# PRBonn/OverlapNet

Measured on AMD Instinct MI355X. Metric: scan-pairs/s (64x900 range images), higher is better.
Workload: dtype f32 (scaled 3-term fp16 split on the fp16 MFMA: 22 significand bits per operand, fp32 accumulate)

## Files before the change

overlapnet_amd/csrc/c3_dense.hip:

```cpp
#include "ovn_internal.h"

typedef _Float16 f16x8 __attribute__((ext_vector_type(8)));
typedef _Float16 f16x4 __attribute__((ext_vector_type(4)));

namespace {

struct ArithF16 {
  typedef _Float16 elem;
  typedef f16x8 v8;
  typedef f16x4 v4;
  static __device__ __forceinline__ f32x4 mfma(v8 a, v8 b, f32x4 c) { return __builtin_amdgcn_mfma_f32_16x16x32_f16(a, b, c, 0, 0, 0); }
};

constexpr int G = OVN_G;
constexpr int OW = OVN_O3_HW;
constexpr int CI = OVN_C2_OUT;
constexpr int CO = OVN_C3_OUT;
constexpr int NBAND = 3;
constexpr int MAX_ROWS = 8;
constexpr int MAX_MT = (MAX_ROWS * OW + 15) / 16;
constexpr int IN_PIX_MAX = (MAX_ROWS + 2) * G;
constexpr int PLANE = IN_PIX_MAX * 8 + 8;
constexpr int NPL = CI / 8;
constexpr size_t LDS_BYTES = 2 * (size_t)NPL * PLANE * sizeof(_Float16) + 64;
constexpr int NW = 8;

__device__ __forceinline__ int band_start(int b) { return b == 0 ? 0 : (b == 1 ? 8 : 15); }
__device__ __forceinline__ int band_rows(int b) { return b == 0 ? 8 : 7; }

constexpr int MT_SPLIT = 6;
template <class A, int NWV, int MSPLIT>
__global__ __launch_bounds__(64 * NWV) void c3_dense_kernel(const float* __restrict__ o2, const typename A::elem* __restrict__ wp,
                                                           const float* __restrict__ b3, const float* __restrict__ wd,
                                                           const unsigned* __restrict__ o2max, float sw3,
                                                           float* __restrict__ partial, float* __restrict__ o3,
                                                           unsigned* __restrict__ arrived, const float* __restrict__ bd,
                                                           float* __restrict__ overlap, float* __restrict__ logit) {
  typedef typename A::elem elem_t;
  typedef typename A::v8 v8_t;
  typedef typename A::v4 v4_t;
  extern __shared__ __attribute__((aligned(16))) unsigned char smem[];
  elem_t* ih = reinterpret_cast<elem_t*>(smem);
  elem_t* il = ih + NPL * PLANE;
  float* red = reinterpret_cast<float*>(il + NPL * PLANE);

  constexpr int HALVES = NW / NWV;
  constexpr int MTW = MSPLIT == 1 ? MAX_MT : MT_SPLIT;
  const int sub = blockIdx.x % (HALVES * MSPLIT);
  const int unit = blockIdx.x / (HALVES * MSPLIT), half = sub % HALVES, mh = sub / HALVES;
  const int mt0 = MT_SPLIT * mh;
  const int pair = unit / NBAND;
  const int band = unit - pair * NBAND;
  const int r0 = band_start(band);
  const int nrows = band_rows(band);
  const int npix = nrows * OW;
  const int nmt = (npix + 15) >> 4;
  const int tid = threadIdx.x;
  const int lane = tid & 63;
  const int wave_l = tid >> 6;
  const int wave = wave_l + NWV * half;
  const int lrow = lane & 15;
  const int g = lane >> 4;

  const elem_t* wsrc = wp + ((size_t)(2 * wave) * 2) * 512 + lane * 8;
  v8_t bq[3][4];
#define C3_LOAD_B(DST, KC)                                                                  \
  {                                                                                         \
    const elem_t* q = wsrc + (size_t)(KC) * (16 * 2 * 512);                                 \
    DST[0] = *reinterpret_cast<const v8_t*>(q);                                           \
    DST[1] = *reinterpret_cast<const v8_t*>(q + 512);                                     \
    DST[2] = *reinterpret_cast<const v8_t*>(q + 1024);                                    \
    DST[3] = *reinterpret_cast<const v8_t*>(q + 1536);                                    \
  }
  C3_LOAD_B(bq[0], 0)
  C3_LOAD_B(bq[1], 1)
  const float s2 = ovn_pow2_scale_for(__uint_as_float(o2max[pair]));
  const float inv = 1.0f / (s2 * sw3);
  {
    const float* src = o2 + ((long long)pair * G + r0) * G * CI;
    const int n4 = (nrows + 2) * G * CI / 4;
    constexpr int PER_THREAD = (MAX_ROWS + 2) * G * CI / 4 / (64 * NWV);
    static_assert(PER_THREAD * 64 * NWV == (MAX_ROWS + 2) * G * CI / 4, "patch does not divide over the threads");
    f32x4 v[PER_THREAD];
#pragma unroll
    for (int k = 0; k < PER_THREAD; ++k) {
      const int i = tid + k * (64 * NWV);
      v[k] = (i < n4) ? *reinterpret_cast<const f32x4*>(src + 4 * i) : (f32x4){0.f, 0.f, 0.f, 0.f};
    }
#pragma unroll
    for (int k = 0; k < PER_THREAD; ++k) {
      const int i = tid + k * (64 * NWV);
      if (i < n4) {
        const int pix = i / (CI / 4);
        const int c = 4 * (i - pix * (CI / 4));
        v4_t h, l;
// ... 58 lines not shown
        C3_READ_A(nb, 1, 2 * q + 3)                                                         \
      } else if (MTW % 2 == 1 && nmt == MAX_MT) {                                                           \
        C3_READ_A(nb, 0, MTW - 1)                                                        \
      }                                                                                     \
      __builtin_amdgcn_sched_barrier(0);   \
      C3_MFMA2(2 * q, 2 * q + 1, fh[cb][0], fl[cb][0], fh[cb][1], fl[cb][1], SRC)           \
      __builtin_amdgcn_sched_barrier(0);                                                    \
    }                                                                                       \
    if (MTW % 2 == 1 && nmt == MAX_MT) {                               \
      const v8_t ah = fh[(MTW / 2) & 1][0], al = fl[(MTW / 2) & 1][0];              \
      acc[MTW - 1][0] = A::mfma(ah, SRC[0], acc[MTW - 1][0]); \
      acc[MTW - 1][1] = A::mfma(ah, SRC[2], acc[MTW - 1][1]); \
      acc[MTW - 1][0] = A::mfma(al, SRC[0], acc[MTW - 1][0]); \
      acc[MTW - 1][1] = A::mfma(al, SRC[2], acc[MTW - 1][1]); \
      acc[MTW - 1][0] = A::mfma(ah, SRC[1], acc[MTW - 1][0]); \
      acc[MTW - 1][1] = A::mfma(ah, SRC[3], acc[MTW - 1][1]); \
    }                                                                                       \
  }
  __syncthreads();
#pragma unroll 1
  for (int kc = 0; kc < 36; kc += 3) {
    C3_LOAD_B(bq[2], kc + 2)
    C3_STEP(bq[0], kc)
    if (kc + 3 < 36) C3_LOAD_B(bq[0], kc + 3)
    C3_STEP(bq[1], kc + 1)
    if (kc + 4 < 36) C3_LOAD_B(bq[1], kc + 4)
    C3_STEP(bq[2], kc + 2)
  }
#undef C3_LOAD_B
#undef C3_STEP
#undef C3_MFMA2
#undef C3_READ_A

  float s[2] = {0.f, 0.f};
#pragma unroll
  for (int nt = 0; nt < 2; ++nt) {
    const int n = 32 * wave + 16 * nt + lrow;
    const float bv = b3[n];
#pragma unroll
    for (int mt = 0; mt < MTW; ++mt) {
#pragma unroll
      for (int r = 0; r < 4; ++r) {
        const int p = 16 * (mt0 + mt) + 4 * g + r;
        if (p < npix) {
          const float v = fmaxf(fmaf(acc[mt][nt][r], inv, bv), 0.0f);
          const long long fi = (long long)(r0 * OW + p) * CO + n;
          s[(MSPLIT == 1 && mt >= MT_SPLIT) ? 1 : 0] += v * wd[fi];
          if (o3) o3[(long long)pair * OVN_DENSE_IN + fi] = v;
        }
      }
    }
  }
#pragma unroll
  for (int off = 32; off > 0; off >>= 1) {
    s[0] += __shfl_down(s[0], off, 64);
    if (MSPLIT == 1) s[1] += __shfl_down(s[1], off, 64);
  }
  if (lane == 0) {
    red[wave_l] = s[0];
    if (MSPLIT == 1) red[NW + wave_l] = s[1];
  }
  __syncthreads();
  if (tid == 0) {
    float* dst = partial + ((size_t)pair * NBAND + band) * 4;
    if (NWV == NW) {
      dst[0] = (red[0] + red[1]) + (red[2] + red[3]);
      dst[1] = (red[NW + 0] + red[NW + 1]) + (red[NW + 2] + red[NW + 3]);
      dst[2] = (red[4] + red[5]) + (red[6] + red[7]);
      dst[3] = (red[NW + 4] + red[NW + 5]) + (red[NW + 6] + red[NW + 7]);
    } else {
      dst[2 * half + mh] = (red[0] + red[1]) + (red[2] + red[3]);
    }
    if (overlap != nullptr) {
      constexpr unsigned PARTS = NBAND * HALVES * MSPLIT;
      __threadfence();
      const unsigned prev = atomicAdd(arrived + pair, 1u);
      if (prev == PARTS - 1) {
        __threadfence();
        const float* q = partial + (size_t)pair * OVN_DENSE_PARTIALS;
        float z = 0.f;
#pragma unroll
        for (int b = 0; b < NBAND; ++b) {
          const float q0 = __hip_atomic_load(q + 4 * b, __ATOMIC_RELAXED, __HIP_MEMORY_SCOPE_AGENT);
          const float q1 = __hip_atomic_load(q + 4 * b + 1, __ATOMIC_RELAXED, __HIP_MEMORY_SCOPE_AGENT);
          const float q2 = __hip_atomic_load(q + 4 * b + 2, __ATOMIC_RELAXED, __HIP_MEMORY_SCOPE_AGENT);
          const float q3 = __hip_atomic_load(q + 4 * b + 3, __ATOMIC_RELAXED, __HIP_MEMORY_SCOPE_AGENT);
          const float zb = (q0 + q1) + (q2 + q3);
          z = b == 0 ? zb : z + zb;
        }
        z += bd[0];
        if (logit) logit[pair] = z;
        overlap[pair] = 1.0f / (1.0f + expf(-z));
        __hip_atomic_store(arrived + pair, 0u, __ATOMIC_RELAXED, __HIP_MEMORY_SCOPE_AGENT);
      }
    }
  }
}

__global__ __launch_bounds__(256) void dense_finish_kernel(const float* __restrict__ partial, const float* __restrict__ bd, int n,
                                                           float* __restrict__ overlap, float* __restrict__ logit) {
  const int p = blockIdx.x * 256 + threadIdx.x;
  if (p >= n) return;
  const float* q = partial + (size_t)p * OVN_DENSE_PARTIALS;
  float z = 0.f;
#pragma unroll
  for (int b = 0; b < NBAND; ++b) {
    const float zb = (q[4 * b] + q[4 * b + 1]) + (q[4 * b + 2] + q[4 * b + 3]);
    z = b == 0 ? zb : z + zb;
  }
  z += bd[0];
  if (logit) logit[p] = z;
  overlap[p] = 1.0f / (1.0f + expf(-z));
}

}

int ovn_c3_dense_forward(const ovn_ctx* ctx, const float* o2, const unsigned* o2max, int n, float* partial, float* o3,
                         unsigned* arrived, float* overlap, float* logit, hipStream_t stream) {
  OVN_REQUIRE(o2max != nullptr, OVN_ERR_ARG, "ovn_c3_dense_forward: the per-pair maxima of o2 are required");
  OVN_REQUIRE(overlap == nullptr || arrived != nullptr, OVN_ERR_ARG, "ovn_c3_dense_forward: arrival counters missing");
  int rc;
  if (n <= 21) {
    rc = ovn_allow_dynamic_lds(reinterpret_cast<const void*>(c3_dense_kernel<ArithF16, 4, 2>), LDS_BYTES);
    if (rc) return rc;
    hipLaunchKernelGGL((c3_dense_kernel<ArithF16, 4, 2>), dim3(4 * NBAND * n), dim3(64 * 4), LDS_BYTES, stream, o2,
                       reinterpret_cast<const _Float16*>(ctx->c3.wp_h), ctx->c3.bias, ctx->wd, o2max, ctx->c3.sw_h, partial, o3, arrived,
                       ctx->bd, overlap, logit);
  } else {
    rc = ovn_allow_dynamic_lds(reinterpret_cast<const void*>(c3_dense_kernel<ArithF16, NW, 1>), LDS_BYTES);
    if (rc) return rc;
    hipLaunchKernelGGL((c3_dense_kernel<ArithF16, NW, 1>), dim3(NBAND * n), dim3(64 * NW), LDS_BYTES, stream, o2,
                       reinterpret_cast<const _Float16*>(ctx->c3.wp_h), ctx->c3.bias, ctx->wd, o2max, ctx->c3.sw_h, partial, o3,
                       (unsigned*)nullptr, ctx->bd, (float*)nullptr, (float*)nullptr);
    if (overlap != nullptr)
      hipLaunchKernelGGL(dense_finish_kernel, dim3((n + 255) / 256), dim3(256), 0, stream, partial, ctx->bd, n, overlap, logit);
  }
  OVN_HIP_CHECK(hipGetLastError());
  return OVN_OK;
}
```

overlapnet_amd/csrc/ovn_api.hip:

```cpp
#include <stdarg.h>
#include <mutex>
#include <set>
#include <utility>
#include <stdio.h>
#include <stdlib.h>
#include <string.h>

#include <algorithm>
#include "ovn_internal.h"

int ovn_allow_dynamic_lds(const void* kernel, size_t bytes) {
  static std::mutex mu;
  static std::set<std::pair<const void*, int>> done;
  int dev = 0;
  OVN_HIP_CHECK(hipGetDevice(&dev));
  std::lock_guard<std::mutex> lock(mu);
  if (done.count({kernel, dev})) return OVN_OK;
  OVN_HIP_CHECK(hipFuncSetAttribute(kernel, hipFuncAttributeMaxDynamicSharedMemorySize, (int)bytes));
  done.insert({kernel, dev});
  return OVN_OK;
}

static thread_local char g_err[1024] = "";

// ... 14 lines not shown
    ctx->dbg_o2 = ctx->dbg_o3 = nullptr;
    ctx->dbg_partial = nullptr;
    ctx->dbg_o2max = nullptr;
    ctx->dbg_n = 0;
    ctx->dbg_live = nullptr;
  }
  const size_t want = bytes + bytes / 8;
  OVN_HIP_CHECK(hipMalloc(&ctx->ws, want));
  ctx->ws_bytes = want;
  return OVN_OK;
}

static int ctx_feat_w(const ovn_ctx* ctx) { return ctx->finalized ? ctx->feat_w : OVN_FEAT_W; }

extern "C" {

int ovn_abi_version(void) { return OVN_ABI_VERSION; }

const char* ovn_last_error(void) { return g_err; }

int ovn_create(int device_id, int in_h, int in_w, int in_c, ovn_ctx** out) {
  OVN_REQUIRE(out != nullptr, OVN_ERR_ARG, "ovn_create: out is NULL");
  OVN_REQUIRE(in_h > 0 && in_w > 0 && in_c > 0, OVN_ERR_ARG, "ovn_create: bad input shape %dx%dx%d", in_h, in_w, in_c);
  int ndev = 0;
  OVN_HIP_CHECK(hipGetDeviceCount(&ndev));
  OVN_REQUIRE(device_id >= 0 && device_id < ndev, OVN_ERR_ARG, "ovn_create: device %d not present (%d devices)", device_id, ndev);
  OVN_ON_DEVICE(device_id);
  hipDeviceProp_t prop;
  OVN_HIP_CHECK(hipGetDeviceProperties(&prop, device_id));
  OVN_REQUIRE(strncmp(prop.gcnArchName, "gfx950", 6) == 0, OVN_ERR_STATE,
              "ovn_create: this library is built for gfx950 only, device %d is %s", device_id, prop.gcnArchName);
  ovn_ctx* c = new ovn_ctx();
  c->device = device_id;
  c->in_h = in_h;
  c->in_w = in_w;
  c->in_c = in_c;
  if (const char* e = getenv("OVN_HEAD_CHUNK")) c->head_chunk = atoll(e) > 0 ? atoll(e) : c->head_chunk;
  if (const char* e = getenv("OVN_HEAD_SUBCHUNK")) c->head_sub = atoll(e) >= 0 ? atoll(e) : c->head_sub;
  if (const char* e = getenv("OVN_HEAD_STREAMS")) c->head_streams = atoi(e) == 2 ? 2 : 1;
  if (const char* e = getenv("OVN_YAW_SIDE")) c->head_yaw_side = atoi(e) ? 1 : 0;
  int rc = ovn_spectral_prepare(c, nullptr);
  if (rc) {
    ovn_conv_release(&c->dft);
    if (c->tw64) (void)hipFree(c->tw64);
    delete c;
    return rc;
  }
  *out = c;
  return OVN_OK;
}

int ovn_destroy(ovn_ctx* ctx) {
  if (!ctx) return OVN_OK;
  if (ctx->comm) (void)ovn_comm_destroy(ctx);
  OVN_ON_DEVICE(ctx->device);
  (void)hipDeviceSynchronize();
  for (auto& l : ctx->leg) ovn_conv_release(&l);
  ovn_conv_release(&ctx->c2);
  ovn_conv_release(&ctx->c3);
  ovn_conv_release(&ctx->dft);
  if (ctx->tw64) (void)hipFree(ctx->tw64);
  if (ctx->w1p) (void)hipFree(ctx->w1p);
  if (ctx->b1) (void)hipFree(ctx->b1);
  if (ctx->wd) (void)hipFree(ctx->wd);
  if (ctx->bd) (void)hipFree(ctx->bd);
  if (ctx->w1p_h) (void)hipFree(ctx->w1p_h);
  if (ctx->w2p_h) (void)hipFree(ctx->w2p_h);
  if (ctx->w1raw) (void)hipFree(ctx->w1raw);
  if (ctx->w1sum) (void)hipFree(ctx->w1sum);
  if (ctx->w1col) (void)hipFree(ctx->w1col);
  if (ctx->wsp_h) (void)hipFree(ctx->wsp_h);
  if (ctx->w2sum) (void)hipFree(ctx->w2sum);
  if (ctx->w1p_b3) (void)hipFree(ctx->w1p_b3);
  if (ctx->w2p_b3) (void)hipFree(ctx->w2p_b3);
  if (ctx->w2raw) (void)hipFree(ctx->w2raw);
  if (ctx->w3raw) (void)hipFree(ctx->w3raw);
  if (ctx->ws) (void)hipFree(ctx->ws);
  if (ctx->norm_buf) (void)hipFree(ctx->norm_buf);
  if (ctx->actmax) (void)hipFree(ctx->actmax);
  if (ctx->c3_arrived) (void)hipFree(ctx->c3_arrived);
  if (ctx->seg_dev) (void)hipFree(ctx->seg_dev);
  if (ctx->seg_host) (void)hipHostFree(ctx->seg_host);
  if (ctx->seg_ev) (void)hipEventDestroy(ctx->seg_ev);
  if (ctx->seg_done) (void)hipEventDestroy(ctx->seg_done);
  if (ctx->aux_ready) {
    for (int i = 0; i < 2; ++i) {
      (void)hipStreamDestroy(ctx->aux[i]);
      (void)hipEventDestroy(ctx->ev_join[i]);
    }
    (void)hipEventDestroy(ctx->ev_fork);
  }
  delete ctx;
  return OVN_OK;
}

static int leg_layer_prepare(OvnConvLayer* L, const float* kernel_dev, const float* bias_dev, hipStream_t stream) {
  int rc = ovn_conv_prepare(L, kernel_dev, bias_dev, stream);
  if (rc == OVN_OK) rc = ovn_conv_prepare_f16x3(L, kernel_dev, stream);
  if (rc == OVN_OK) {
    const size_t bytes = (size_t)L->kh * L->kw * L->cin * L->cout * sizeof(float);
    hipError_t e = hipMalloc((void**)&L->wraw, bytes);
    if (e == hipSuccess) e = hipMemcpyAsync(L->wraw, kernel_dev, bytes, hipMemcpyDeviceToDevice, stream);
    if (e == hipSuccess) e = hipStreamSynchronize(stream);
    if (e != hipSuccess) {
      ovn_set_error("layer %s: keeping the raw kernel failed: %s", L->name.c_str(), hipGetErrorString(e));
      rc = OVN_ERR_HIP;
    }
  }
  if (rc) ovn_conv_release(L);
  return rc;
}

int ovn_add_leg_layer(ovn_ctx* ctx, const char* name, const float* kernel_dev, const float* bias_dev, int kh, int kw,
// ... 17 lines not shown
  int rc = leg_layer_prepare(&L, kernel_dev, bias_dev, (hipStream_t)stream);
  if (rc) return rc;
  ctx->leg.push_back(L);
  return OVN_OK;
}

int ovn_set_leg_layer_weights(ovn_ctx* ctx, int layer, const float* kernel_dev, const float* bias_dev, void* stream) {
  OVN_REQUIRE(ctx && kernel_dev && bias_dev, OVN_ERR_ARG, "ovn_set_leg_layer_weights: NULL argument");
  OVN_REQUIRE(ctx->finalized, OVN_ERR_STATE, "ovn_set_leg_layer_weights: context not finalized");
  OVN_REQUIRE(layer >= 0 && layer < (int)ctx->leg.size(), OVN_ERR_ARG, "ovn_set_leg_layer_weights: no such leg layer %d", layer);
  OVN_ON_DEVICE(ctx->device);
  OvnConvLayer N = ctx->leg[layer];
  N.wp = N.bias = N.wraw = nullptr;
  N.wp_h = N.wp_h16 = nullptr;
  N.sw_h = 1.f;
  int rc = leg_layer_prepare(&N, kernel_dev, bias_dev, (hipStream_t)stream);
  if (rc) return rc;
  ovn_conv_release(&ctx->leg[layer]);
  ctx->leg[layer] = N;
  return OVN_OK;
}

int ovn_set_head_weights(ovn_ctx* ctx, const float* c1k, const float* c1b, const float* c2k, const float* c2b,
                         const float* c3k, const float* c3b, const float* dk, const float* db, void* stream_) {
  OVN_REQUIRE(ctx && c1k && c1b && c2k && c2b && c3k && c3b && dk && db, OVN_ERR_ARG, "ovn_set_head_weights: NULL argument");
  OVN_ON_DEVICE(ctx->device);
  hipStream_t stream = (hipStream_t)stream_;
  {
    ovn_conv_release(&ctx->c2);
    ovn_conv_release(&ctx->c3);
    if (ctx->w1p) (void)hipFree(ctx->w1p);
    if (ctx->b1) (void)hipFree(ctx->b1);
    if (ctx->wd) (void)hipFree(ctx->wd);
    if (ctx->bd) (void)hipFree(ctx->bd);
    if (ctx->w1p_h) (void)hipFree(ctx->w1p_h);
    if (ctx->w2p_h) (void)hipFree(ctx->w2p_h);
    if (ctx->w1raw) (void)hipFree(ctx->w1raw);
    if (ctx->w1sum) (void)hipFree(ctx->w1sum);
    if (ctx->w1col) (void)hipFree(ctx->w1col);
    if (ctx->wsp_h) (void)hipFree(ctx->wsp_h);
      if (ctx->w2sum) (void)hipFree(ctx->w2sum);
    if (ctx->w1p_b3) (void)hipFree(ctx->w1p_b3);
    if (ctx->w2p_b3) (void)hipFree(ctx->w2p_b3);
    if (ctx->w2raw) (void)hipFree(ctx->w2raw);
    if (ctx->w3raw) (void)hipFree(ctx->w3raw);
    ctx->w3raw = nullptr;
    ctx->w1p_h = ctx->w2p_h = ctx->wsp_h = ctx->w1p_b3 = ctx->w2p_b3 = nullptr;
    ctx->w1raw = ctx->w1sum = ctx->w1col = ctx->w2sum = ctx->w2raw = nullptr;
    ctx->w1p = ctx->b1 = ctx->wd = ctx->bd = nullptr;
    ctx->head_set = false;
  }
  ctx->head_g = ctx_feat_w(ctx) / ctx->head_s;
  const int hs = ctx->head_s, hg = ctx->head_g;
  OVN_REQUIRE(hg >= 3, OVN_ERR_ARG, "ovn_set_head_weights: conv1size %d leaves %d column groups, c_conv3 needs 3", hs, hg);
  const bool general = (hs != OVN_S);
  int rc = OVN_OK;
  if (!general) {
    rc = ovn_delta_prepare_w1(c1k, &ctx->w1p, stream);
    if (rc) return rc;
  } else {
    const size_t w1_bytes = (size_t)hs * OVN_FEAT_C * OVN_C1_OUT * sizeof(float);
    OVN_HIP_CHECK(hipMalloc((void**)&ctx->w1raw, w1_bytes));
    OVN_HIP_CHECK(hipMemcpyAsync(ctx->w1raw, c1k, w1_bytes, hipMemcpyDeviceToDevice, stream));
  }
  OVN_HIP_CHECK(hipMalloc((void**)&ctx->b1, OVN_C1_OUT * sizeof(float)));
  OVN_HIP_CHECK(hipMemcpyAsync(ctx->b1, c1b, OVN_C1_OUT * sizeof(float), hipMemcpyDeviceToDevice, stream));
  ctx->c2 = OvnConvLayer();
  ctx->c2.name = "c_conv2";
  ctx->c2.kh = hs;
  ctx->c2.kw = 1;
  ctx->c2.cin = OVN_C1_OUT;
  ctx->c2.cout = OVN_C2_OUT;
  ctx->c2.sh = hs;
  ctx->c2.sw = 1;
  ctx->c2.relu = 1;
  rc = ovn_conv_prepare(&ctx->c2, c2k, c2b, stream);
  if (rc) return rc;
  if (!general) {
    rc = ovn_delta_prepare_f16x3(ctx, c1k, c1b, c2k, stream);
    if (rc) return rc;
  }
  ctx->c3 = OvnConvLayer();
  ctx->c3.name = "c_conv3";
  ctx->c3.kh = 3;
  ctx->c3.kw = 3;
  ctx->c3.cin = OVN_C2_OUT;
  ctx->c3.cout = OVN_C3_OUT;
  ctx->c3.sh = 1;
  ctx->c3.sw = 1;
  ctx->c3.relu = 1;
  rc = ovn_conv_prepare(&ctx->c3, c3k, c3b, stream);
  if (rc) return rc;
  if (!general) {
    rc = ovn_conv_prepare_f16x3(&ctx->c3, c3k, stream);
    if (rc) return rc;
  }
  const size_t w3_bytes = (size_t)9 * OVN_C2_OUT * OVN_C3_OUT * sizeof(float);
  OVN_HIP_CHECK(hipMalloc((void**)&ctx->w3raw, w3_bytes));
  OVN_HIP_CHECK(hipMemcpyAsync(ctx->w3raw, c3k, w3_bytes, hipMemcpyDeviceToDevice, stream));
  if (!ctx->w2raw) {
    const size_t w2_bytes = (size_t)hs * OVN_C1_OUT * OVN_C2_OUT * sizeof(float);
    OVN_HIP_CHECK(hipMalloc((void**)&ctx->w2raw, w2_bytes));
    OVN_HIP_CHECK(hipMemcpyAsync(ctx->w2raw, c2k, w2_bytes, hipMemcpyDeviceToDevice, stream));
  }
  const size_t dense_in = (size_t)(hg - 2) * (hg - 2) * OVN_C3_OUT;
  OVN_HIP_CHECK(hipMalloc((void**)&ctx->wd, dense_in * sizeof(float)));
  OVN_HIP_CHECK(hipMalloc((void**)&ctx->bd, sizeof(float)));
  OVN_HIP_CHECK(hipMemcpyAsync(ctx->wd, dk, dense_in * sizeof(float), hipMemcpyDeviceToDevice, stream));
  OVN_HIP_CHECK(hipMemcpyAsync(ctx->bd, db, sizeof(float), hipMemcpyDeviceToDevice, stream));
  OVN_HIP_CHECK(hipStreamSynchronize(stream));
  ctx->head_set = true;
  return OVN_OK;
}

int ovn_finalize(ovn_ctx* ctx, int* feat_w) {
  OVN_REQUIRE(ctx != nullptr, OVN_ERR_ARG, "ovn_finalize: ctx is NULL");
  OVN_REQUIRE(!ctx->leg.empty(), OVN_ERR_STATE, "ovn_finalize: no leg layers registered");
  int h = ctx->in_h, w = ctx->in_w, c = ctx->in_c;
  for (const auto& l : ctx->leg) {
    OVN_REQUIRE(h >= l.kh && w >= l.kw, OVN_ERR_ARG, "ovn_finalize: layer %s does not fit its %dx%d input", l.name.c_str(), h, w);
    h = (h - l.kh) / l.sh + 1;
    w = (w - l.kw) / l.sw + 1;
    c = l.cout;
  }
  OVN_REQUIRE(h == 1 && w >= OVN_FEAT_W_MIN && w <= OVN_FEAT_W_MAX && c == OVN_FEAT_C, OVN_ERR_ARG,
              "ovn_finalize: leg produces %dx%dx%d, the heads need 1 x W x %d with %d <= W <= %d", h, w, c, OVN_FEAT_C, OVN_FEAT_W_MIN,
              OVN_FEAT_W_MAX);
  OVN_REQUIRE(!ctx->head_set || w / ctx->head_s == ctx->head_g, OVN_ERR_STATE,
              "ovn_finalize: leg width %d gives %d column groups, the head weights were registered for %d", w, w / ctx->head_s,
              ctx->head_g);
  ctx->feat_w = w;
  ctx->finalized = true;
  if (feat_w) *feat_w = w;
  return OVN_OK;
}

int ovn_leg(ovn_ctx* ctx, const float* images_dev, int64_t n, float* features_dev, void* stream_) {
  OVN_REQUIRE(ctx && ctx->finalized, OVN_ERR_STATE, "ovn_leg: context not finalized");
  OVN_REQUIRE(n >= 0, OVN_ERR_ARG, "ovn_leg: n < 0");
  if (n == 0) return OVN_OK;
  OVN_REQUIRE(images_dev && features_dev, OVN_ERR_ARG, "ovn_leg: NULL buffer");
  OVN_ON_DEVICE(ctx->device);
// ... 433 lines not shown
                            ridx ? ridx + c0 : nullptr, (int)cn, fw, yaw + c0, corr ? corr + (size_t)c0 * fw : nullptr, stream,
                            ctx->corr_norm);
      if (rc) return rc;
    }
    int j = 0;
    for (int64_t q0 = 0; q0 < cn; q0 += sub, ++j) {
      const int64_t p0 = c0 + q0;
      const int np = (int)((cn - q0 < sub) ? (cn - q0) : sub);
      hipStream_t st = stream;
      if (nstreams == 2 && (j & 1)) {
        rc = fk.side(0, &st);
        if (rc) return rc;
      }
      const float* fl = lidx ? feats_l : feats_l + (size_t)p0 * feat_elems;
      const int32_t* li = lidx ? lidx + p0 : nullptr;
      const int32_t* ri = ridx ? ridx + p0 : nullptr;
      float* o2s = o2 + (size_t)q0 * o2_elems;
      if (fused) {
        unsigned* o2max = nullptr;
        float* part = o3 + (size_t)q0 * OVN_DENSE_PARTIALS;
        OvnSegPass sp{};
        if (seg) {
          sp = *seg;
          sp.pseg += p0;
          sp.scratch = dscratch + sc_sub * nsub_max;
        }
        rc = ovn_delta_c12_f16x3_forward(ctx, fl, li, feats_r, ri, np, dscratch + (size_t)j * sc_sub, &o2max, o2s, st, (int)(p0 & 0x3fffffff),
                                          dcache_l ? (lidx ? dcache_l : dcache_l + (size_t)p0 * OVN_DELTA_CACHE_ELEMS) : nullptr, a2_in_yaw,
                                          seg ? &sp : nullptr);
        if (rc) return rc;
        if (p0 == 0) ctx->dbg_o2max = o2max;
        {
          OvnProfScope ps(ctx, OVN_K_C3, st);
          rc = ovn_c3_dense_forward(ctx, o2s, o2max, np, part, nullptr, ctx->c3_arrived + q0, overlap + p0, logit ? logit + p0 : nullptr, st);
        }
      } else {
        float* o3s = o3 + (size_t)q0 * o3_elems;
        rc = ovn_delta_c12_bf16x3_forward(ctx, fl, li, feats_r, ri, np, dscratch + (size_t)j * sc_sub, o2s, st, (int)(p0 & 0x3fffffff),
                                          a2_in_yaw);
        if (rc) return rc;
        int oh = 0, ow = 0;
        {
          OvnProfScope ps(ctx, OVN_K_C3, st);
          rc = ovn_conv_forward(ctx->c3, o2s, np, OVN_G, OVN_G, o3s, &oh, &ow, st);
        }
        if (rc) return rc;
        OvnProfScope ps(ctx, OVN_K_DENSE, st);
        rc = ovn_dense_sigmoid_forward(ctx, o3s, np, OVN_DENSE_IN, overlap + p0, logit ? logit + p0 : nullptr, st);
      }
      if (rc) return rc;
    }
  }
  return fk.join();
}

int ovn_heads(ovn_ctx* ctx, const float* feats_l, const int32_t* lidx, const float* feats_r, const int32_t* ridx,
              int64_t n, float* overlap, int32_t* yaw, float* logit, float* corr, void* stream_) {
  OVN_REQUIRE(ctx && ctx->head_set, OVN_ERR_STATE, "ovn_heads: head weights not set");
  OVN_REQUIRE(n >= 0 && n < (1ll << 31), OVN_ERR_ARG, "ovn_heads: bad n");
  if (n == 0) return OVN_OK;
  OVN_REQUIRE(feats_l && feats_r && overlap && yaw, OVN_ERR_ARG, "ovn_heads: NULL buffer");
  OVN_ON_DEVICE(ctx->device);
  return delta_head_run(ctx, feats_l, lidx, feats_r, ridx, n, overlap, logit, yaw, corr, 1, nullptr, nullptr, nullptr, (hipStream_t)stream_);
}

int ovn_heads_spectral(ovn_ctx* ctx, const float* feats_l, const float* spec_l, const float* dcache_l, const int32_t* lidx,
                       const float* feats_r, const float* spec_r, const int32_t* ridx, int64_t n, float* overlap, int32_t* yaw,
// ... 481 lines not shown
    (void)hipEventDestroy(r.b);
  }
  ctx->prof_recs.clear();
  return rc;
}

int ovn_debug_conv(ovn_ctx* ctx, int layer, const float* in_dev, int nb, int h, int w, float* out_dev, void* stream) {
  OVN_REQUIRE(ctx && layer >= 0 && layer < (int)ctx->leg.size(), OVN_ERR_ARG, "ovn_debug_conv: no such leg layer");
  OVN_REQUIRE(in_dev && out_dev && nb >= 0, OVN_ERR_ARG, "ovn_debug_conv: bad buffers");
  OVN_ON_DEVICE(ctx->device);
  int oh = 0, ow = 0;
  if (ctx->leg_mode == 0) return ovn_conv_forward(ctx->leg[layer], in_dev, nb, h, w, out_dev, &oh, &ow, (hipStream_t)stream);
  OVN_REQUIRE(nb <= OVN_LEG_SLICE, OVN_ERR_ARG, "ovn_debug_conv: at most %d images per call", OVN_LEG_SLICE);
  if (!ctx->actmax) OVN_HIP_CHECK(hipMalloc((void**)&ctx->actmax, (size_t)OVN_ACTMAX_SLOTS * OVN_LEG_SLICE * OVN_ACTMAX_STRIDE * sizeof(unsigned)));
  OVN_HIP_CHECK(hipMemsetAsync(ctx->actmax, 0, 2 * (size_t)OVN_LEG_SLICE * OVN_ACTMAX_STRIDE * sizeof(unsigned), (hipStream_t)stream));
  int rc = ovn_absmax_forward(in_dev, nb, (long long)h * w * ctx->leg[layer].cin, ctx->actmax, (hipStream_t)stream);
  if (rc) return rc;
  return ovn_conv_forward_f16x3(ctx->leg[layer], in_dev, nb, h, w, out_dev, &oh, &ow, ctx->actmax, ctx->actmax + (size_t)OVN_LEG_SLICE * OVN_ACTMAX_STRIDE,
                                (hipStream_t)stream);
}

int ovn_debug_head_activations(ovn_ctx* ctx, int64_t n, float* o2_dev, float* o3_dev, void* stream) {
  OVN_REQUIRE(ctx && ctx->dbg_o2 && n >= 0 && n <= ctx->dbg_n, OVN_ERR_STATE,
              "ovn_debug_head_activations: call right after ovn_heads with n <= its (first-chunk) pair count");
  OVN_ON_DEVICE(ctx->device);
  const size_t g = (size_t)ctx->head_g;
  if (o2_dev)
    OVN_HIP_CHECK(hipMemcpyAsync(o2_dev, ctx->dbg_o2, (size_t)n * g * g * OVN_C2_OUT * sizeof(float),
                                 hipMemcpyDeviceToDevice, (hipStream_t)stream));
  if (o3_dev && ctx->dbg_o3)
    OVN_HIP_CHECK(hipMemcpyAsync(o3_dev, ctx->dbg_o3, (size_t)n * (g - 2) * (g - 2) * OVN_C3_OUT * sizeof(float),
                                 hipMemcpyDeviceToDevice, (hipStream_t)stream));
  else if (o3_dev)
    return ovn_c3_dense_forward(ctx, ctx->dbg_o2, ctx->dbg_o2max, (int)n, ctx->dbg_partial, o3_dev, nullptr, nullptr, nullptr, (hipStream_t)stream);
  return OVN_OK;
}

int ovn_head_walk_stats(ovn_ctx* ctx, int32_t* out16_host, void* stream) {
  OVN_REQUIRE(ctx && out16_host, OVN_ERR_ARG, "ovn_head_walk_stats: NULL argument");
  OVN_ON_DEVICE(ctx->device);
  return ovn_delta_walk_stats(ctx, out16_host, (hipStream_t)stream);
}

int64_t ovn_workspace_bytes(ovn_ctx* ctx) { return ctx ? (int64_t)ctx->ws_bytes : 0; }

int ovn_selftest(ovn_ctx* ctx) {
  OVN_REQUIRE(ctx != nullptr, OVN_ERR_ARG, "ovn_selftest: ctx is NULL");
  OVN_ON_DEVICE(ctx->device);
  return ovn_mfma_selftest(nullptr);
}

}
```

overlapnet_amd/csrc/ovn_internal.h:

```cpp
#pragma once

#include <hip/hip_runtime.h>
#include <math.h>
#include <stdint.h>

#include <string>
#include <vector>

#include "../../include/ovn_hip.h"

typedef float f32x4 __attribute__((ext_vector_type(4)));

void ovn_set_error(const char* fmt, ...);

#define OVN_HIP_CHECK(expr)                                                                   \
  do {                                                                                        \
    hipError_t _e = (expr);                                                                   \
    if (_e != hipSuccess) {                                                                   \
      ovn_set_error("%s failed: %s (%s:%d)", #expr, hipGetErrorString(_e), __FILE__, __LINE__); \
      return OVN_ERR_HIP;                                                                     \
    }                                                                                         \
  } while (0)

#define OVN_REQUIRE(cond, code, ...)   \
// ... 185 lines not shown

struct ovn_ctx {
  int device = 0;
  int in_h = 0, in_w = 0, in_c = 0;
  std::vector<OvnConvLayer> leg;
  bool finalized = false;
  int feat_w = 0;
  bool head_set = false;
  int head_s = OVN_S;
  int head_g = OVN_G;
  float* w1p = nullptr;
  float* b1 = nullptr;
  OvnConvLayer c2;
  OvnConvLayer c3;
  void* w1p_h = nullptr;
  void* w2p_h = nullptr;
  float* w1raw = nullptr;
  float* w1sum = nullptr;
  float* w1col = nullptr;
  void* wsp_h = nullptr;
  float* w2sum = nullptr;
  void* w1p_b3 = nullptr;
  void* w2p_b3 = nullptr;
  float* w2raw = nullptr;
  float* w3raw = nullptr;
  OvnHeadScales hs;
  int leg_mode = 1;
  int head_compact = 1;
  int proj_trig = 0;
  unsigned* actmax = nullptr;
  int head_mode = 1;
  int head_width_split = 0;
  float* wd = nullptr;
  float* bd = nullptr;
  OvnConvLayer dft;
  double* tw64 = nullptr;
  int corr_norm = 0;
  float* norm_buf = nullptr;
  int64_t norm_buf_n = 0;
  void* comm = nullptr;
  int comm_rank = 0, comm_world = 1;
  int64_t head_chunk = 1024;
  int64_t head_sub = 0;
  int head_streams = 1;
  int head_yaw_side = 0;
  bool aux_ready = false;
  hipStream_t aux[2] = {nullptr, nullptr};
  hipEvent_t ev_fork = nullptr, ev_join[2] = {nullptr, nullptr};
  void* ws = nullptr;
  size_t ws_bytes = 0;
  bool prof = false;
  struct ProfRec {
    hipEvent_t a, b;
    int kind;
  };
  std::vector<ProfRec> prof_recs;
  const float* dbg_o2 = nullptr;
  const float* dbg_o3 = nullptr;
  float* dbg_partial = nullptr;
  const unsigned* dbg_o2max = nullptr;
  int64_t dbg_n = 0;
  unsigned* c3_arrived = nullptr;
  int64_t c3_arrived_n = 0;
  const unsigned* dbg_live = nullptr;
  void* seg_host = nullptr;
  void* seg_dev = nullptr;
  size_t seg_cap = 0;
  hipEvent_t seg_ev = nullptr;
  hipEvent_t seg_done = nullptr;
  bool seg_ev_pending = false;
};

enum { OVN_K_LEG = 0, OVN_K_CORR = 1, OVN_K_DELTA = 2, OVN_K_C3 = 3, OVN_K_DENSE = 4, OVN_K_PROJ = 5, OVN_K_SPECTRUM = 6,
       OVN_K_CORR_SPECTRAL = 7, OVN_K_DELTA_PREP = 8, OVN_K_DELTA_C2 = 9, OVN_K_COUNT = 10 };

struct OvnProfScope {
  ovn_ctx* ctx;
  hipStream_t stream;
  hipEvent_t a = nullptr, b = nullptr;
  int kind;
  OvnProfScope(ovn_ctx* c, int k, hipStream_t s) : ctx(c), stream(s), kind(k) {
    if (ctx->prof && hipEventCreate(&a) == hipSuccess && hipEventCreate(&b) == hipSuccess) (void)hipEventRecord(a, stream);
  }
  ~OvnProfScope() {
    if (ctx->prof && a && b) {
      (void)hipEventRecord(b, stream);
      ctx->prof_recs.push_back({a, b, kind});
    }
  }
};

int ovn_ws_reserve(ovn_ctx* ctx, size_t bytes, hipStream_t stream);

int ovn_conv_prepare(OvnConvLayer* L, const float* kernel_dev, const float* bias_dev, hipStream_t stream);
void ovn_conv_release(OvnConvLayer* L);
int ovn_conv_forward(const OvnConvLayer& L, const float* in, int nb, int h, int w, float* out, int* oh,
// ... 50 lines not shown
int ovn_delta_data_grad(ovn_ctx* ctx, int FW, const float* feats_l, const int32_t* lidx, const float* feats_r, const int32_t* ridx,
                        const float* dO1, int np, float* dfeat_l, float* dfeat_r, hipStream_t stream);
int ovn_yaw_grad_run(ovn_ctx* ctx, int FW, const float* feats_l, const int32_t* lidx, const float* feats_r, const int32_t* ridx,
                     int64_t n, const float* target, const int32_t* yaw_bin, float yaw_scale, float thr, float* dfeat_l, float* dfeat_r,
                     float* loss_yaw, float* corr, hipStream_t stream);

size_t ovn_leg_grad_part_bytes(const OvnConvLayer& L, int h, int w, int nb);
int ovn_leg_mask_forward(const float* dy, const float* y, float* out, long long n, hipStream_t stream);
int ovn_leg_grad_round(const double* acc, float* out, long long n, hipStream_t stream);
int ovn_leg_layer_backward(const OvnConvLayer& L, const float* x, const float* dym, int nb, int h, int w, float* dx, const float* mask,
                           double* acc_kernel, double* acc_bias, double* part, hipStream_t stream);

size_t ovn_delta_w_split_pair_bytes();
int ovn_delta_w_split_c12_forward(ovn_ctx* ctx, const float* feats_l, const int32_t* lidx, const float* feats_r, const int32_t* ridx,
                                  int n, void* scales, float* o2, hipStream_t stream);

int ovn_corr_forward(const float* feats_l, const int32_t* lidx, const float* feats_r, const int32_t* ridx, int n, int W,
                     int32_t* yaw, float* corr, hipStream_t stream, int norm_mode);

int ovn_spectral_prepare(ovn_ctx* ctx, hipStream_t stream);
int ovn_spectrum_forward(ovn_ctx* ctx, const float* feats, int n, float* spectra, hipStream_t stream);
bool ovn_conv_strip_own_scale(const OvnConvLayer& L, long long call_nb, int h, int w);
int ovn_conv_strip_try(const OvnConvLayer& L, const float* in, int nb, long long call_nb, int h, int w, float* out,
                       const unsigned* in_max, unsigned* out_max, hipStream_t stream);

bool ovn_leg_front_matches(const ovn_ctx* ctx, size_t first, int h, int w);
int ovn_leg_front_forward(const ovn_ctx* ctx, size_t first, const float* in, int nb, int h, int w, float* out, int* oh_out, int* ow_out,
                          unsigned* out_max, hipStream_t stream);

bool ovn_leg_tail_matches(const ovn_ctx* ctx, size_t first, int h, int w);
int ovn_leg_tail_forward(const ovn_ctx* ctx, size_t first, const float* in, int nb, int w, float* out, hipStream_t stream);

int ovn_c3_dense_forward(const ovn_ctx* ctx, const float* o2, const unsigned* o2max, int n, float* partial, float* o3,
                         unsigned* arrived, float* overlap, float* logit, hipStream_t stream);

int ovn_gt_range_forward(const float* points, const int64_t* offsets, int n_scans, long long max_points, const double* ref_poses,
                         const double* inv_cur_pose, int H, int W, double fov_up_deg, double fov_down_deg, double max_range,
                         float* range_out, hipStream_t stream);
int ovn_gt_count_forward(const float* ref_ranges, const float* cur_range, int n, int npix, int32_t* counts, hipStream_t stream);
int ovn_gt_pair_forward(const float* points, const int64_t* offsets, int n_scans, const double* poses, const double* inv_poses,
                        const float* cur_ranges, const int32_t* frame_idx, int n_frames, const int32_t* ref_idx, int n_refs, int H,
                        int W, double fov_up_deg, double fov_down_deg, double max_range, int frame_fastest, int32_t* counts,
                        hipStream_t stream);
int ovn_best_match_forward(const float* overlap, const int32_t* yaw, const int32_t* ids, int n, float threshold,
                           int index_offset, int32_t* out, hipStream_t stream);
int ovn_top_k_forward(const float* overlap, const int32_t* yaw, const int32_t* ids, int n, int k, float threshold,
                      int index_offset, int32_t* out, hipStream_t stream);
int ovn_top_k_segments_forward(const float* overlap, const int32_t* yaw, const int32_t* ids, const int64_t* offs_dev, int B, int k,
                               float threshold, int32_t* out, hipStream_t stream);
int ovn_segment_ridx_forward(const int64_t* offs_dev, const int32_t* qidx_dev, int B, int n, int32_t* ridx, int32_t* pseg,
                             hipStream_t stream);
int ovn_corr_spectral_forward(ovn_ctx* ctx, const float* spec_l, const int32_t* lidx, const float* spec_r,
                              const int32_t* ridx, int n, int32_t* yaw, float* corr, hipStream_t stream,
                              const float* a2_feats_r = nullptr, float* a2raw = nullptr);

int ovn_project_forward(ovn_ctx* ctx, const float* points, const int64_t* offsets, int n_scans,
                        int64_t max_points, int H, int W, double fov_up_deg, double fov_down_deg,
                        double max_range, float* range, float* vertex, float* intensity, int32_t* idx,
                        float* normal, float* stacked, int use_depth, int use_normals, int use_intensity,
                        hipStream_t stream);

int ovn_project_semantic_forward(ovn_ctx* ctx, const float* points, const int64_t* offsets, int n_scans, int64_t max_points, int H,
                                 int W, double fov_up_deg, double fov_down_deg, double max_range, const float* probs, int n_classes,
                                 float* range, float* vertex, float* intensity, int32_t* idx, float* normal, float* semantic,
                                 int32_t* sem_idx, float* stacked, int use_depth, int use_normals, int use_semantic, int use_intensity,
                                 hipStream_t stream);
int ovn_projection_angles_forward(const float* points, int64_t n, int H, int W, double fov_up_deg, double fov_down_deg,
// ... 6 lines not shown
```

Baseline: 239,200.

## Make c3 dense kernel persistent with atomic work claiming and lane-ordered dense weights

For large batches the c3+dense kernel now launches one block per CU, and each block claims (pair, band) units through an atomic counter until the work runs out. The next unit is prefetched while the epilogue runs. Dense weights are re-laid out once at head setup into a per-lane f32x4 order, so the epilogue issues coalesced vector loads that are double-buffered instead of scattered scalar loads. The o3 debug store is split into a separate loop. This adds a memset and an atomic per unit, and relies on one resident 512-thread block per CU being enough to keep the CU busy.

```diff
diff --git a/overlapnet_amd/csrc/c3_dense.hip b/overlapnet_amd/csrc/c3_dense.hip
--- a/overlapnet_amd/csrc/c3_dense.hip
+++ b/overlapnet_amd/csrc/c3_dense.hip
@@ -22,8 +22,9 @@
 constexpr int IN_PIX_MAX = (MAX_ROWS + 2) * G;
 constexpr int PLANE = IN_PIX_MAX * 8 + 8;
 constexpr int NPL = CI / 8;
-constexpr size_t LDS_BYTES = 2 * (size_t)NPL * PLANE * sizeof(_Float16) + 64;
+constexpr size_t LDS_BYTES = 2 * (size_t)NPL * PLANE * sizeof(_Float16) + 64 + 16;
 constexpr int NW = 8;
+constexpr int WD_LANE_ELEMS = NBAND * NW * 2 * MAX_MT * 64 * 4;
 
 __device__ __forceinline__ int band_start(int b) { return b == 0 ? 0 : (b == 1 ? 8 : 15); }
 __device__ __forceinline__ int band_rows(int b) { return b == 0 ? 8 : 7; }
@@ -31,11 +32,12 @@
 constexpr int MT_SPLIT = 6;
 template <class A, int NWV, int MSPLIT>
 __global__ __launch_bounds__(64 * NWV) void c3_dense_kernel(const float* __restrict__ o2, const typename A::elem* __restrict__ wp,
-                                                           const float* __restrict__ b3, const float* __restrict__ wd,
+                                                           const float* __restrict__ b3, const float* __restrict__ wd_lane,
                                                            const unsigned* __restrict__ o2max, float sw3,
                                                            float* __restrict__ partial, float* __restrict__ o3,
                                                            unsigned* __restrict__ arrived, const float* __restrict__ bd,
-                                                           float* __restrict__ overlap, float* __restrict__ logit) {
+                                                           float* __restrict__ overlap, float* __restrict__ logit,
+                                                           unsigned* __restrict__ claim, unsigned nunits) {
   typedef typename A::elem elem_t;
   typedef typename A::v8 v8_t;
   typedef typename A::v4 v4_t;
@@ -43,24 +45,36 @@
   elem_t* ih = reinterpret_cast<elem_t*>(smem);
   elem_t* il = ih + NPL * PLANE;
   float* red = reinterpret_cast<float*>(il + NPL * PLANE);
-
+  unsigned* claimed = reinterpret_cast<unsigned*>(red + 2 * NW);
+
+  constexpr bool RESIDENT = (NWV == NW && MSPLIT == 1);
   constexpr int HALVES = NW / NWV;
   constexpr int MTW = MSPLIT == 1 ? MAX_MT : MT_SPLIT;
   const int sub = blockIdx.x % (HALVES * MSPLIT);
-  const int unit = blockIdx.x / (HALVES * MSPLIT), half = sub % HALVES, mh = sub / HALVES;
+  const int half = sub % HALVES, mh = sub / HALVES;
   const int mt0 = MT_SPLIT * mh;
+  unsigned unit = blockIdx.x / (HALVES * MSPLIT);
+  if (RESIDENT) {
+    if (threadIdx.x == 0) *claimed = atomicAdd(claim, 1u);
+    __syncthreads();
+    unit = __builtin_amdgcn_readfirstlane(*claimed);
+    if (unit >= nunits) return;
+  }
+#pragma unroll 1
+  do {
+  int tid = threadIdx.x;
+  if (RESIDENT) asm volatile("" : "+v"(tid));
+  const int lane = tid & 63;
+  const int wave_l = tid >> 6;
+  const int wave = wave_l + NWV * half;
+  const int lrow = lane & 15;
+  const int g = lane >> 4;
   const int pair = unit / NBAND;
   const int band = unit - pair * NBAND;
   const int r0 = band_start(band);
   const int nrows = band_rows(band);
   const int npix = nrows * OW;
   const int nmt = (npix + 15) >> 4;
-  const int tid = threadIdx.x;
-  const int lane = tid & 63;
-  const int wave_l = tid >> 6;
-  const int wave = wave_l + NWV * half;
-  const int lrow = lane & 15;
-  const int g = lane >> 4;
 
   const elem_t* wsrc = wp + ((size_t)(2 * wave) * 2) * 512 + lane * 8;
   v8_t bq[3][4];
@@ -185,22 +199,57 @@
 #undef C3_MFMA2
 #undef C3_READ_A
 
+  constexpr int NH = (MTW + MT_SPLIT - 1) / MT_SPLIT;
+  const f32x4* wl = reinterpret_cast<const f32x4*>(wd_lane) + ((size_t)((band * NW + wave) * 2) * MAX_MT + mt0) * 64 + lane;
+  const float bv2[2] = {b3[32 * wave + lrow], b3[32 * wave + 16 + lrow]};
+  f32x4 wq[2][MT_SPLIT];
+#define C3_LOAD_W(BUF, GI)                                                                  \
+  _Pragma("unroll") for (int j = 0; j < MT_SPLIT; ++j) {                                    \
+    const int mt = ((GI) % NH) * MT_SPLIT + j;                                              \
+    if (mt < MTW)                                                                           \
+      wq[BUF][j] = (MSPLIT == 1 || mt0 + mt < MAX_MT) ? wl[(((GI) / NH) * MAX_MT + mt) * 64] : (f32x4){0.f, 0.f, 0.f, 0.f};   \
+  }
+  C3_LOAD_W(0, 0)
+  unsigned next_unit = 0;
+  if (RESIDENT && tid == 0) next_unit = atomicAdd(claim, 1u);
   float s[2] = {0.f, 0.f};
 #pragma unroll
-  for (int nt = 0; nt < 2; ++nt) {
-    const int n = 32 * wave + 16 * nt + lrow;
-    const float bv = b3[n];
-#pragma unroll
-    for (int mt = 0; mt < MTW; ++mt) {
-#pragma unroll
-      for (int r = 0; r < 4; ++r) {
-        const int p = 16 * (mt0 + mt) + 4 * g + r;
-        if (p < npix) {
-          const float v = fmaxf(fmaf(acc[mt][nt][r], inv, bv), 0.0f);
-          const long long fi = (long long)(r0 * OW + p) * CO + n;
-          s[(MSPLIT == 1 && mt >= MT_SPLIT) ? 1 : 0] += v * wd[fi];
-          if (o3) o3[(long long)pair * OVN_DENSE_IN + fi] = v;
+  for (int gi = 0; gi < 2 * NH; ++gi) {
+    const int nt = gi / NH, h = gi % NH;
+    if (gi + 1 < 2 * NH) C3_LOAD_W((gi + 1) & 1, gi + 1)
+    __builtin_amdgcn_sched_barrier(0);
+    const float bv = bv2[nt];
+#pragma unroll
+    for (int j = 0; j < MT_SPLIT; ++j) {
+      const int mt = h * MT_SPLIT + j;
+      if (mt < MTW) {
+#pragma unroll
+        for (int r = 0; r < 4; ++r) {
+          const int p = 16 * (mt0 + mt) + 4 * g + r;
+          if (p < npix) {
+            const float v = fmaxf(fmaf(acc[mt][nt][r], inv, bv), 0.0f);
+            s[(MSPLIT == 1 && mt >= MT_SPLIT) ? 1 : 0] += v * wq[gi & 1][j][r];
+          }
         }
+      }
+    }
+    __builtin_amdgcn_sched_barrier(0);
+  }
+#undef C3_LOAD_W
+  if (o3 != nullptr) {
+    float* o3p = o3 + (long long)pair * OVN_DENSE_IN + (long long)(r0 * OW + 4 * g) * CO + 32 * wave + lrow;
+    asm volatile("" : "+v"(o3p));
+#pragma unroll
+    for (int nt = 0; nt < 2; ++nt) {
+      const float bv = bv2[nt];
+#pragma unroll
+      for (int mt = 0; mt < MTW; ++mt) {
+#pragma unroll
+        for (int r = 0; r < 4; ++r) {
+          const int p = 16 * (mt0 + mt) + 4 * g + r;
+          if (p < npix) o3p[(16 * (mt0 + mt) + r) * CO + 16 * nt] = fmaxf(fmaf(acc[mt][nt][r], inv, bv), 0.0f);
+        }
+        __builtin_amdgcn_sched_barrier(0);
       }
     }
   }
@@ -213,6 +262,7 @@
     red[wave_l] = s[0];
     if (MSPLIT == 1) red[NW + wave_l] = s[1];
   }
+  if (RESIDENT && tid == 0) *claimed = next_unit;
   __syncthreads();
   if (tid == 0) {
     float* dst = partial + ((size_t)pair * NBAND + band) * 4;
@@ -248,6 +298,23 @@
       }
     }
   }
+  if (RESIDENT) unit = __builtin_amdgcn_readfirstlane(*claimed);
+  } while (RESIDENT && unit < nunits);
+}
+
+__global__ __launch_bounds__(256) void wd_lane_kernel(const float* __restrict__ wd, float* __restrict__ out) {
+  const int i = blockIdx.x * 256 + threadIdx.x;
+  if (i >= WD_LANE_ELEMS) return;
+  const int r = i & 3, lane = (i >> 2) & 63;
+  int t = i >> 8;
+  const int mt = t % MAX_MT;
+  t /= MAX_MT;
+  const int nt = t & 1;
+  t >>= 1;
+  const int wave = t % NW, band = t / NW;
+  const int n = 32 * wave + 16 * nt + (lane & 15);
+  const int p = 16 * mt + 4 * (lane >> 4) + r;
+  out[i] = p < band_rows(band) * OW ? wd[(size_t)(band_start(band) * OW + p) * CO + n] : 0.0f;
 }
 
 __global__ __launch_bounds__(256) void dense_finish_kernel(const float* __restrict__ partial, const float* __restrict__ bd, int n,
@@ -268,23 +335,38 @@
 
 }
 
+int ovn_c3_dense_prepare(ovn_ctx* ctx, hipStream_t stream) {
+  OVN_REQUIRE(ctx->wd != nullptr, OVN_ERR_STATE, "ovn_c3_dense_prepare: the Dense kernel is not registered");
+  if (!ctx->wd_lane) OVN_HIP_CHECK(hipMalloc((void**)&ctx->wd_lane, (size_t)WD_LANE_ELEMS * sizeof(float)));
+  if (!ctx->c3_claim) OVN_HIP_CHECK(hipMalloc((void**)&ctx->c3_claim, 2 * sizeof(unsigned)));
+  hipLaunchKernelGGL(wd_lane_kernel, dim3((WD_LANE_ELEMS + 255) / 256), dim3(256), 0, stream, ctx->wd, ctx->wd_lane);
+  OVN_HIP_CHECK(hipGetLastError());
+  return OVN_OK;
+}
+
 int ovn_c3_dense_forward(const ovn_ctx* ctx, const float* o2, const unsigned* o2max, int n, float* partial, float* o3,
-                         unsigned* arrived, float* overlap, float* logit, hipStream_t stream) {
+                         unsigned* arrived, unsigned* claim, float* overlap, float* logit, hipStream_t stream) {
   OVN_REQUIRE(o2max != nullptr, OVN_ERR_ARG, "ovn_c3_dense_forward: the per-pair maxima of o2 are required");
+  OVN_REQUIRE(ctx->wd_lane != nullptr, OVN_ERR_STATE, "ovn_c3_dense_forward: the Dense kernel is not laid out (24 x 24 heads only)");
+  OVN_REQUIRE(n > 0 && n <= (1 << 29), OVN_ERR_ARG, "ovn_c3_dense_forward: bad n %d", n);
   OVN_REQUIRE(overlap == nullptr || arrived != nullptr, OVN_ERR_ARG, "ovn_c3_dense_forward: arrival counters missing");
   int rc;
   if (n <= 21) {
     rc = ovn_allow_dynamic_lds(reinterpret_cast<const void*>(c3_dense_kernel<ArithF16, 4, 2>), LDS_BYTES);
     if (rc) return rc;
     hipLaunchKernelGGL((c3_dense_kernel<ArithF16, 4, 2>), dim3(4 * NBAND * n), dim3(64 * 4), LDS_BYTES, stream, o2,
-                       reinterpret_cast<const _Float16*>(ctx->c3.wp_h), ctx->c3.bias, ctx->wd, o2max, ctx->c3.sw_h, partial, o3, arrived,
-                       ctx->bd, overlap, logit);
+                       reinterpret_cast<const _Float16*>(ctx->c3.wp_h), ctx->c3.bias, ctx->wd_lane, o2max, ctx->c3.sw_h, partial, o3, arrived,
+                       ctx->bd, overlap, logit, (unsigned*)nullptr, 0u);
   } else {
-    rc = ovn_allow_dynamic_lds(reinterpret_cast<const void*>(c3_dense_kernel<ArithF16, NW, 1>), LDS_BYTES);
+    OVN_REQUIRE(claim != nullptr && ctx->num_cus > 0, OVN_ERR_ARG, "ovn_c3_dense_forward: unit counter missing");
+    auto kernel = c3_dense_kernel<ArithF16, NW, 1>;
+    rc = ovn_allow_dynamic_lds(reinterpret_cast<const void*>(kernel), LDS_BYTES);
     if (rc) return rc;
-    hipLaunchKernelGGL((c3_dense_kernel<ArithF16, NW, 1>), dim3(NBAND * n), dim3(64 * NW), LDS_BYTES, stream, o2,
-                       reinterpret_cast<const _Float16*>(ctx->c3.wp_h), ctx->c3.bias, ctx->wd, o2max, ctx->c3.sw_h, partial, o3,
-                       (unsigned*)nullptr, ctx->bd, (float*)nullptr, (float*)nullptr);
+    const int nunits = NBAND * n;
+    OVN_HIP_CHECK(hipMemsetAsync(claim, 0, sizeof(unsigned), stream));
+    hipLaunchKernelGGL(kernel, dim3(nunits < ctx->num_cus ? nunits : ctx->num_cus), dim3(64 * NW), LDS_BYTES, stream, o2,
+                       reinterpret_cast<const _Float16*>(ctx->c3.wp_h), ctx->c3.bias, ctx->wd_lane, o2max, ctx->c3.sw_h, partial, o3,
+                       (unsigned*)nullptr, ctx->bd, (float*)nullptr, (float*)nullptr, claim, (unsigned)nunits);
     if (overlap != nullptr)
       hipLaunchKernelGGL(dense_finish_kernel, dim3((n + 255) / 256), dim3(256), 0, stream, partial, ctx->bd, n, overlap, logit);
   }
diff --git a/overlapnet_amd/csrc/ovn_api.hip b/overlapnet_amd/csrc/ovn_api.hip
--- a/overlapnet_amd/csrc/ovn_api.hip
+++ b/overlapnet_amd/csrc/ovn_api.hip
@@ -70,6 +70,7 @@
               "ovn_create: this library is built for gfx950 only, device %d is %s", device_id, prop.gcnArchName);
   ovn_ctx* c = new ovn_ctx();
   c->device = device_id;
+  c->num_cus = prop.multiProcessorCount;
   c->in_h = in_h;
   c->in_w = in_w;
   c->in_c = in_c;
@@ -101,6 +102,7 @@
   if (ctx->w1p) (void)hipFree(ctx->w1p);
   if (ctx->b1) (void)hipFree(ctx->b1);
   if (ctx->wd) (void)hipFree(ctx->wd);
+  if (ctx->wd_lane) (void)hipFree(ctx->wd_lane);
   if (ctx->bd) (void)hipFree(ctx->bd);
   if (ctx->w1p_h) (void)hipFree(ctx->w1p_h);
   if (ctx->w2p_h) (void)hipFree(ctx->w2p_h);
@@ -117,6 +119,7 @@
   if (ctx->norm_buf) (void)hipFree(ctx->norm_buf);
   if (ctx->actmax) (void)hipFree(ctx->actmax);
   if (ctx->c3_arrived) (void)hipFree(ctx->c3_arrived);
+  if (ctx->c3_claim) (void)hipFree(ctx->c3_claim);
   if (ctx->seg_dev) (void)hipFree(ctx->seg_dev);
   if (ctx->seg_host) (void)hipHostFree(ctx->seg_host);
   if (ctx->seg_ev) (void)hipEventDestroy(ctx->seg_ev);
@@ -200,6 +203,7 @@
     if (ctx->w1p) (void)hipFree(ctx->w1p);
     if (ctx->b1) (void)hipFree(ctx->b1);
     if (ctx->wd) (void)hipFree(ctx->wd);
+    if (ctx->wd_lane) (void)hipFree(ctx->wd_lane);
     if (ctx->bd) (void)hipFree(ctx->bd);
     if (ctx->w1p_h) (void)hipFree(ctx->w1p_h);
     if (ctx->w2p_h) (void)hipFree(ctx->w2p_h);
@@ -215,7 +219,7 @@
     ctx->w3raw = nullptr;
     ctx->w1p_h = ctx->w2p_h = ctx->wsp_h = ctx->w1p_b3 = ctx->w2p_b3 = nullptr;
     ctx->w1raw = ctx->w1sum = ctx->w1col = ctx->w2sum = ctx->w2raw = nullptr;
-    ctx->w1p = ctx->b1 = ctx->wd = ctx->bd = nullptr;
+    ctx->w1p = ctx->b1 = ctx->wd = ctx->wd_lane = ctx->bd = nullptr;
     ctx->head_set = false;
   }
   ctx->head_g = ctx_feat_w(ctx) / ctx->head_s;
@@ -276,6 +280,10 @@
   OVN_HIP_CHECK(hipMalloc((void**)&ctx->bd, sizeof(float)));
   OVN_HIP_CHECK(hipMemcpyAsync(ctx->wd, dk, dense_in * sizeof(float), hipMemcpyDeviceToDevice, stream));
   OVN_HIP_CHECK(hipMemcpyAsync(ctx->bd, db, sizeof(float), hipMemcpyDeviceToDevice, stream));
+  if (hg == OVN_G) {
+    rc = ovn_c3_dense_prepare(ctx, stream);
+    if (rc) return rc;
+  }
   OVN_HIP_CHECK(hipStreamSynchronize(stream));
   ctx->head_set = true;
   return OVN_OK;
@@ -775,7 +783,7 @@
         if (p0 == 0) ctx->dbg_o2max = o2max;
         {
           OvnProfScope ps(ctx, OVN_K_C3, st);
-          rc = ovn_c3_dense_forward(ctx, o2s, o2max, np, part, nullptr, ctx->c3_arrived + q0, overlap + p0, logit ? logit + p0 : nullptr, st);
+          rc = ovn_c3_dense_forward(ctx, o2s, o2max, np, part, nullptr, ctx->c3_arrived + q0, ctx->c3_claim + (st == stream ? 0 : 1), overlap + p0, logit ? logit + p0 : nullptr, st);
         }
       } else {
         float* o3s = o3 + (size_t)q0 * o3_elems;
@@ -1323,7 +1331,8 @@
     OVN_HIP_CHECK(hipMemcpyAsync(o3_dev, ctx->dbg_o3, (size_t)n * (g - 2) * (g - 2) * OVN_C3_OUT * sizeof(float),
                                  hipMemcpyDeviceToDevice, (hipStream_t)stream));
   else if (o3_dev)
-    return ovn_c3_dense_forward(ctx, ctx->dbg_o2, ctx->dbg_o2max, (int)n, ctx->dbg_partial, o3_dev, nullptr, nullptr, nullptr, (hipStream_t)stream);
+    return ovn_c3_dense_forward(ctx, ctx->dbg_o2, ctx->dbg_o2max, (int)n, ctx->dbg_partial, o3_dev, nullptr, ctx->c3_claim, nullptr, nullptr,
+                                (hipStream_t)stream);
   return OVN_OK;
 }
 
diff --git a/overlapnet_amd/csrc/ovn_internal.h b/overlapnet_amd/csrc/ovn_internal.h
--- a/overlapnet_amd/csrc/ovn_internal.h
+++ b/overlapnet_amd/csrc/ovn_internal.h
@@ -241,6 +241,7 @@
   int head_mode = 1;
   int head_width_split = 0;
   float* wd = nullptr;
+  float* wd_lane = nullptr;
   float* bd = nullptr;
   OvnConvLayer dft;
   double* tw64 = nullptr;
@@ -271,6 +272,8 @@
   int64_t dbg_n = 0;
   unsigned* c3_arrived = nullptr;
   int64_t c3_arrived_n = 0;
+  unsigned* c3_claim = nullptr;
+  int num_cus = 0;
   const unsigned* dbg_live = nullptr;
   void* seg_host = nullptr;
   void* seg_dev = nullptr;
@@ -387,7 +390,8 @@
 int ovn_leg_tail_forward(const ovn_ctx* ctx, size_t first, const float* in, int nb, int w, float* out, hipStream_t stream);
 
 int ovn_c3_dense_forward(const ovn_ctx* ctx, const float* o2, const unsigned* o2max, int n, float* partial, float* o3,
-                         unsigned* arrived, float* overlap, float* logit, hipStream_t stream);
+                         unsigned* arrived, unsigned* claim, float* overlap, float* logit, hipStream_t stream);
+int ovn_c3_dense_prepare(ovn_ctx* ctx, hipStream_t stream);
 
 int ovn_gt_range_forward(const float* points, const int64_t* offsets, int n_scans, long long max_points, const double* ref_poses,
                          const double* inv_cur_pose, int H, int W, double fov_up_deg, double fov_down_deg, double max_range,
```

New measurement: 241,000, median of 6. About the same (+0.7%).
